# Dont4rootMe/beast_tokenizer

Measured on AMD Instinct MI355X. Metric: trajectories/sec encode+reconstruct (B=4096,T=50,DoF=14), higher is better.
Workload: dtype f32 (fp32 MFMA fit, int64 tokens); 1 GPU; BEASTBsplineTokenizer encode->reconstruct_traj, num_dof=14 num_basis=10 seq_len=50 vocab=256 degree_p=4; global_batch=4096, per_gpu_batch=4096, seq_len=50, parallelism=dp1

## Files before the change

### beast_tokenizer_amd/csrc/codec.hip

```cpp
#include <hip/hip_runtime.h>

#include <atomic>

#include <algorithm>
#include <cstdlib>

#include "common.h"
#include "launch.h"
#include "codec_device.h"
#include "codec_encode.h"
#include "codec_reconstruct.h"
#include "codec_roundtrip.h"

namespace {

constexpr int MAX_T = 256;
constexpr int MAX_N = 16;
constexpr int MAX_D = 64;

bool g_generic_only = false;

int g_block_waves = 0;
bool wide_blocks(int64_t ntiles, const Queue& q) {
  if (g_block_waves == 4 || g_block_waves == 7 || g_block_waves == 8) return g_block_waves != 4;
// ... 67 lines not shown
    case 2: return enc_smem<2>(T, Tp, Dl, D, N, nkinds).total;
    case 4: return enc_smem<4>(T, Tp, Dl, D, N, nkinds).total;
    default: return enc_smem<8>(T, Tp, Dl, D, N, nkinds).total;
  }
}

int launch_encode(EncArgs a, int T, int D, int nj, int N, const Queue& q) {
  const int64_t traj_bytes = (int64_t)T * a.row_elems * 4;
  const bool contiguous = a.sd == 1 && a.st == a.row_elems && a.sb == (int64_t)T * a.row_elems &&
                          (((uintptr_t)a.traj) & 15) == 0 && ((int64_t)T * a.row_elems) % 4 == 0;
  static const int forced = [] {
    const char* e = getenv("BEAST_ENC_TBT");
    return e ? atoi(e) : 0;
  }();
  int tbt = 8;
  while (tbt > 1 && tbt * traj_bytes > 32 * 1024) tbt >>= 1;
  const bool fast = contiguous && tbt * traj_bytes <= 32 * 1024;
  if (!fast) {
    tbt = 8;
    while (tbt > 1 && enc_smem_total(tbt, T, D, D, N, nj < D ? 2 : 1) > 160 * 1024) tbt >>= 1;
  }
  if (forced == 1 || forced == 2 || forced == 4 || (forced == 8 && fast)) tbt = std::min(tbt, forced);
  BEAST_REQUIRE(!a.traj_list || (fast && a.list_rows % tbt == 0),
                "encode list: rows must be contiguous and rows per batch a multiple of %d", tbt);
  if (fast && tbt == 8 && !g_generic_only && T == 50 && N == 10 && a.row_elems == D) {
    int rc = 0;
    const bool out16 = (((uintptr_t)a.params_out | (uintptr_t)a.tokens_out) & 15) == 0;
    if (!a.traj_list && enc_v() && out16 &&
        with_fixed_shape<false>(D, nj, false, rc, [&](auto sh) { return launch_encode_v<decltype(sh)>(a, q); }))
      return rc;
    if (with_fixed_shape<true>(D, nj, wide_blocks((a.B + 7) / 8, q), rc, [&](auto sh) {
          return launch_encode_t<8, decltype(sh)>(a, T, D, nj, N, true, q);
        }))
      return rc;
  }
  switch (tbt) {
    case 1: return launch_encode_t<1, DynShape>(a, T, D, nj, N, fast, q);
    case 2: return launch_encode_t<2, DynShape>(a, T, D, nj, N, fast, q);
    case 4: return launch_encode_t<4, DynShape>(a, T, D, nj, N, fast, q);
    default: return launch_encode_t<8, DynShape>(a, T, D, nj, N, fast, q);
  }
}

template <int TBT, int KS, int RT, class S = DynShape>
int launch_rec_ks(RecArgs a, int D, int nj, const Queue& q) {
  const RecSmem L = rec_smem<TBT, KS, RT>(a.Tout, D, a.g.N, a.ndo, nj < D ? 2 : 1, a.lut_n);
  BEAST_REQUIRE_CODE(L.total <= 160 * 1024, BEAST_E_UNSUPPORTED, "reconstruct tile needs %d B of LDS", L.total);
  const int64_t grid = grid_for(a.ntiles, L.total, q.dev);
  if constexpr (KS == 0) {
    mark_launch(launch_mark(FAM_REC_ROWS, TBT, NWAVES, 0, false, false, L.stage, false));
    return launch<k_reconstruct_rows<TBT>>((unsigned)grid, NTHREADS, L.total, q, "k_reconstruct_rows", a);
  } else {
    mark_launch(launch_mark(S::fixed ? FAM_REC_SPEC : FAM_REC_MFMA, TBT, S::W, KS, false, RT > 0, true, S::W == 7));
    return launch<k_reconstruct<TBT, KS, RT, S>>(
        (unsigned)grid, S::W * 64, L.total, q, "k_reconstruct",
        a.ntokens ? static_cast<const void*>(a.ntokens) : static_cast<const void*>(a.tokens), a.B, a.ntokens ? 4 : 8, a);
  }
}

template <int TBT, int RT>
int launch_rec_mfma(RecArgs a, int D, int nj, int N, const Queue& q) {
  switch ((N + 3) / 4) {
    case 1: return launch_rec_ks<TBT, 1, RT>(a, D, nj, q);
    case 2: return launch_rec_ks<TBT, 2, RT>(a, D, nj, q);
    case 3: return launch_rec_ks<TBT, 3, RT>(a, D, nj, q);
    default: return launch_rec_ks<TBT, 4, RT>(a, D, nj, q);
  }
}

bool rec_v(const RecArgs& a, const Queue& q) {
  return (g_block_waves == 8 || (g_block_waves == 0 && a.ntiles <= 2 * (int64_t)cu_count(q.dev))) &&
         a.params_out == nullptr && a.ntokens == nullptr && (((uintptr_t)a.pos_out) & 15) == 0;
}

template <class S>
int launch_rec_v(RecArgs a, const Queue& q) {
  constexpr int KS = (S::N + 3) / 4;
  constexpr RvSmem L = rv_smem<S>(S::NJ < S::D ? 2 : 1);
  static_assert(L.total <= (RV_WR <= 8 ? 64 : 160) * 1024, "k_reconstruct_v LDS");
  a.tbt = RV_WR;
  a.ntiles = (a.B + RV_WR - 1) / RV_WR;
  const bool lat = a.B <= 16 * (int64_t)cu_count(q.dev);
  mark_launch(launch_mark(FAM_REC_V, RV_WR, RV_WR, KS, false, true, true, lat));
  const RecVArgs v{a.w_min, a.w_max, a.basis, a.dof_dst, a.init_p, a.init_p_src, a.pos_out, a.tok_offset,
                   a.init_p_sb, a.vocab, a.lut_n, a.phases};
  const unsigned grid = (unsigned)a.ntiles;
  return lat ? launch<k_reconstruct_v<KS, S, LAT_SP>>(grid, RV_WR * 64, L.total, q, "k_reconstruct_v", a.tokens, a.B, 8, v)
             : launch<k_reconstruct_v<KS, S, 0>>(grid, RV_WR * 64, L.total, q, "k_reconstruct_v", a.tokens, a.B, 8, v);
}

template <int TBT>
bool rec_mfma_fits(int Tout, int D, int N, int ndo, int lut_n) {
  return rec_smem<TBT, 4, 0>(Tout, D, N, ndo, 2, lut_n).total <= 112 * 1024;
}

template <int TBT>
int launch_reconstruct(RecArgs a, int D, int nj, int N, bool shared, const Queue& q) {
  a.g = make_geom<TBT>(D, nj, N, 1);
  a.ntiles = (a.B + TBT - 1) / TBT;
  a.tbt = TBT;
  a.fd_row = make_fd((uint32_t)(a.Tout * a.ndo));
  a.lut_n = (a.ntokens == nullptr && a.vocab <= LUT_MAX) ? a.vocab : 0;
  const bool pos = a.pos_out != nullptr;
  const bool mfma = shared && pos && rec_mfma_fits<TBT>(a.Tout, D, N, a.ndo, a.lut_n);
  if (!mfma) return launch_rec_ks<TBT, 0, 0>(a, D, nj, q);
  if (a.Tout <= 16 * RT_REG) {
    if (!g_generic_only && N == 10 && a.Tout == 50 && a.ndo == D) {
      int rc = 0;
      const bool wide = wide_blocks(a.ntiles, q);
      if (wide && rec_v(a, q) &&
          with_fixed_shape<false>(D, nj, false, rc, [&](auto sh) { return launch_rec_v<decltype(sh)>(a, q); }))
        return rc;
      if (with_fixed_shape<true>(D, nj, wide, rc, [&](auto sh) {
            return launch_rec_ks<TBT, 3, RT_REG, decltype(sh)>(a, D, nj, q);
          }))
        return rc;
    }
    return launch_rec_mfma<TBT, RT_REG>(a, D, nj, N, q);
  }
  return launch_rec_mfma<TBT, 0>(a, D, nj, N, q);
}

template <class S, int WF>
int launch_roundtrip(const float* traj, int64_t B, RtArgs a, int W, const Queue& q) {
  const RtSmem L = rt_smem(a.T, a.D, a.N, a.nj < a.D ? 2 : 1, W, a.lut_n);
  BEAST_REQUIRE_CODE(L.total <= 160 * 1024, BEAST_E_UNSUPPORTED, "round trip tile needs %d B of LDS", L.total);
  const int64_t grid = grid_for((B + W - 1) / W, L.total, q.dev);
  return launch<k_roundtrip<S, WF>>((unsigned)grid, (unsigned)(W * 64), (unsigned)L.total, q, "k_roundtrip", traj, B, a);
}

template <class S>
int launch_roundtrip_fixed(const float* traj, int64_t B, const RtArgs& a, const Queue& q) {
  return B <= RT_W * (int64_t)cu_count(q.dev) ? launch_roundtrip<S, RT_W>(traj, B, a, RT_W, q)
                                              : launch_roundtrip<S, RT_W_BULK>(traj, B, a, RT_W_BULK, q);
}

}

extern "C" int beast_encode_f32(const float* traj, int64_t B, int T, int64_t sb, int64_t st, int64_t sd,
                                int row_elems, int D, int n_joint, const int32_t* dof_src, const float* proj,
                                int N, const float* w_min, const float* w_max, int vocab, int64_t tok_offset,
                                float* params_out, int64_t* tokens_out, void* stream) {
  BEAST_REQUIRE(traj && dof_src && proj, "beast_encode_f32: null input pointer");
  BEAST_REQUIRE(params_out || tokens_out, "beast_encode_f32: no output requested");
  BEAST_REQUIRE(T >= 1 && T <= MAX_T, "seq_len T=%d outside [1, %d]", T, MAX_T);
  BEAST_REQUIRE(N >= 1 && N <= MAX_N, "num_basis N=%d outside [1, %d]", N, MAX_N);
  BEAST_REQUIRE(D >= 1 && D <= MAX_D && n_joint >= 0 && n_joint <= D, "bad DoF split D=%d n_joint=%d", D, n_joint);
  BEAST_REQUIRE(row_elems >= 1, "row_elems must be >= 1");
  BEAST_REQUIRE(!tokens_out || (w_min && w_max && vocab >= 2), "quantisation needs w_min/w_max and vocab >= 2");
  BEAST_REQUIRE(B >= 0, "batch size B=%lld must be >= 0", (long long)B);
  if (B == 0) return BEAST_OK;
  EncArgs a{};
  a.traj = traj; a.B = B; a.sb = sb; a.st = st; a.sd = sd; a.row_elems = row_elems; a.vocab = vocab;
  a.phases = debug_phases(); a.dof_src = dof_src; a.proj = proj; a.w_min = w_min; a.w_max = w_max;
  a.tok_offset = tok_offset; a.params_out = params_out; a.tokens_out = reinterpret_cast<long long*>(tokens_out);
  Queue q;
  if (const int rc = queue_of(stream, q, "beast_encode_f32")) return rc;
  return launch_encode(a, T, D, n_joint, N, q);
}

extern "C" int beast_encode_list_f32(const float* const* traj_list, int nbatch, int64_t rows_per_batch, int T,
                                     int row_elems, int D, int n_joint, const int32_t* dof_src, const float* proj,
                                     int N, float* params_out, void* stream) {
  BEAST_REQUIRE(traj_list && dof_src && proj && params_out, "beast_encode_list_f32: null pointer");
  BEAST_REQUIRE(nbatch >= 0 && rows_per_batch >= 0, "beast_encode_list_f32: negative sizes");
  BEAST_REQUIRE(rows_per_batch % 8 == 0, "rows_per_batch=%lld is not a multiple of 8", (long long)rows_per_batch);
  BEAST_REQUIRE(T >= 1 && T <= MAX_T, "seq_len T=%d outside [1, %d]", T, MAX_T);
  BEAST_REQUIRE(N >= 1 && N <= MAX_N, "num_basis N=%d outside [1, %d]", N, MAX_N);
// ... 139 lines not shown
```

### beast_tokenizer_amd/csrc/codec_device.h

```cpp
#pragma once

#include <hip/hip_runtime.h>

#include <algorithm>
#include <cstdint>
#include <type_traits>

#include "common.h"

namespace {

constexpr int NTHREADS = 256;
constexpr int NWAVES = NTHREADS / 64;

typedef float float4_t __attribute__((ext_vector_type(4)));

__host__ __device__ constexpr int round_up(int x, int m) { return (x + m - 1) / m * m; }

struct FastDiv {
  uint32_t d, m;
};
inline FastDiv make_fd(uint32_t d) {
  FastDiv f;
  f.d = d;
// ... 21 lines not shown
__device__ __forceinline__ void st16(void* p, float4 v) {
  st16<SP>(p, u32x4_t{__float_as_uint(v.x), __float_as_uint(v.y), __float_as_uint(v.z), __float_as_uint(v.w)});
}
template <int SP>
__device__ __forceinline__ void st16(void* p, long long a, long long b) {
  st16<SP>(p, u32x4_t{(unsigned)a, (unsigned)((unsigned long long)a >> 32), (unsigned)b,
                      (unsigned)((unsigned long long)b >> 32)});
}

template <int NT = NTHREADS, int SP = 0>
__device__ __forceinline__ void store_out(float* __restrict__ dst, const float* __restrict__ src, int count) {
  if ((((uintptr_t)src | (uintptr_t)dst) & 15) == 0) {
    const int n4 = count >> 2;
    const float4* s4 = reinterpret_cast<const float4*>(src);
    float4* d4 = reinterpret_cast<float4*>(dst);
    for (int i = threadIdx.x; i < n4; i += NT) st16<SP>(d4 + i, s4[i]);
    for (int i = (n4 << 2) + threadIdx.x; i < count; i += NT) dst[i] = src[i];
  } else {
    for (int i = threadIdx.x; i < count; i += NT) dst[i] = src[i];
  }
}

typedef __attribute__((address_space(3))) void lds_void;

template <int NT = NTHREADS>
__device__ __forceinline__ void dma16(void* lds, const void* g, int n16) {
  const int tid = threadIdx.x, wb = tid & ~63;
  for (int base = 0; base < n16; base += NT) {
    if (base + wb < n16)
      __builtin_amdgcn_global_load_lds(static_cast<const uint4*>(g) + min(base + tid, n16 - 1),
                                       (lds_void*)(static_cast<uint4*>(lds) + base + wb), 16, 0, 0);
  }
}

template <int NT = NTHREADS>
__device__ __forceinline__ void dma4(void* lds, const void* g, int n) {
  const int tid = threadIdx.x, wb = tid & ~63;
  for (int base = 0; base < n; base += NT) {
    if (base + wb < n)
      __builtin_amdgcn_global_load_lds(static_cast<const uint32_t*>(g) + min(base + tid, n - 1),
                                       (lds_void*)(static_cast<uint32_t*>(lds) + base + wb), 4, 0, 0);
  }
}

template <class V>
__device__ __forceinline__ void pin(V& v) {
  asm volatile("" : "+v"(v));
}

template <int NT = NTHREADS>
__device__ __forceinline__ void stage_rows(void* lds, const void* base, int64_t B, int esz, int64_t b0, int per,
                                           int tbt) {
  const int nb = (int)min<int64_t>(B - b0, tbt);
  const char* src = static_cast<const char*>(base) + b0 * per * esz;
  const int bytes = nb * per * esz;
  if ((bytes & 15) == 0 && (((uintptr_t)src) & 15) == 0) dma16<NT>(lds, src, bytes >> 4);
  else dma4<NT>(lds, src, bytes >> 2);
}


using beast::wave_sync;

__device__ __forceinline__ void lut_fill(float* lut, int lut_n, float vm1, int nt) {
  for (int t = threadIdx.x; t < lut_n; t += nt) lut[t] = __fdiv_rn((float)t, vm1);
}

__device__ __forceinline__ float tok_f32(long long t) { return (float)t; }

template <int NQ, class Tok>
__device__ __forceinline__ void lut_quotients(const Tok (&t)[NQ], const float* lut, int lut_n, float vm1,
                                              float (&nrm)[NQ]) {
  using U = std::make_unsigned_t<Tok>;
  bool far = false;
#pragma unroll
  for (int u = 0; u < NQ; ++u) {
    const bool in = (U)t[u] < (U)lut_n;
    far = far | !in;
    nrm[u] = lut[in ? (int)t[u] : 0];
  }
  if (far) {
#pragma unroll
    for (int u = 0; u < NQ; ++u)
      if (!((U)t[u] < (U)lut_n)) nrm[u] = __fdiv_rn(tok_f32(t[u]), vm1);
  }
}

template <bool Q3>
__device__ __forceinline__ int slot_row(int lk, int u) {
  return (!Q3 || u < 2 || lk < 2) ? (4 * lk | u) : 4 * (lk - 2) + 3;
}
template <bool Q3, int NQ>
__device__ __forceinline__ void slot_values(const float (&p4)[4], float (&p)[NQ]) {
  if constexpr (Q3) {
    const auto sw = __builtin_amdgcn_permlane32_swap(__float_as_uint(p4[2]), __float_as_uint(p4[3]), false, false);
    p[0] = p4[0]; p[1] = p4[1]; p[2] = __uint_as_float(sw[0]);
  } else {
#pragma unroll
    for (int r = 0; r < 4; ++r) p[r] = p4[r];
  }
}

template <int SP, int N16, class T>
__device__ __forceinline__ void wave_copy_out(T* g, const T* img, int lane) {
  constexpr int K = 16 / sizeof(T);
#pragma unroll
  for (int u = 0; u < (N16 + 63) / 64; ++u) {
    const int i = u * 64 + lane;
    if (i < N16) st16<SP>(g + K * i, *reinterpret_cast<const u32x4_t*>(img + K * i));
  }
}

#ifdef BEAST_STAMPS
__device__ unsigned long long g_stamps[2][16][16];
#define STAMP(k, i)                                                                              \
  do {                                                                                           \
    if (blockIdx.x == 0 && (threadIdx.x & 63) == 0) g_stamps[k][threadIdx.x >> 6][i] = __builtin_amdgcn_s_memtime(); \
  } while (0)
__device__ unsigned long long g_bstamps[2][4096][4];
#define BSTAMP(k, i)                                                                             \
  do {                                                                                           \
    if (threadIdx.x == 0 && blockIdx.x < 4096) {                                                 \
      g_bstamps[k][blockIdx.x][i] = __builtin_amdgcn_s_memrealtime();                            \
      if (i == 0)                                                                                \
        g_bstamps[k][blockIdx.x][2] = ((unsigned long long)__builtin_amdgcn_s_getreg(0xF814) << 32) | \
                                      (unsigned)__builtin_amdgcn_s_getreg(0xF804);               \
    }                                                                                            \
  } while (0)
#else
#define STAMP(k, i) do { } while (0)
#define BSTAMP(k, i) do { } while (0)
#endif

struct Geom {
  int D, nj, N, T, Tp, per;
  int nq0, nq;
  FastDiv fd_nj, fd_ng, fd_per, fd_N, fd_D, fd_nq;
};

template <int TBT>
inline Geom make_geom(int D, int nj, int N, int T) {
  Geom g;
  g.D = D; g.nj = nj; g.N = N; g.T = T; g.Tp = round_up(T, 4); g.per = N * D;
  const int ng = D - nj;
  g.nq0 = (TBT * nj + 15) / 16;
  g.nq = g.nq0 + (TBT * ng + 15) / 16;
  g.fd_nj = make_fd(std::max(nj, 1));
  g.fd_ng = make_fd(std::max(ng, 1));
  g.fd_per = make_fd(g.per);
  g.fd_N = make_fd(N);
  g.fd_D = make_fd(D);
  g.fd_nq = make_fd(std::max(g.nq, 1));
  return g;
}

template <int SD, int SNJ, int SN, int ST, int SDL, int SW = NWAVES>
struct Shape {
  static constexpr int D = SD, NJ = SNJ, N = SN, T = ST, DL = SDL;
  static constexpr int W = SW;
  static constexpr bool fixed = SD > 0;
};
using DynShape = Shape<0, 0, 0, 0, 0>;

template <class S>
struct Dims {
  int D, nj, ng, N, T, Tp, per;
  __device__ __forceinline__ Dims(const Geom& g)
// ... 38 lines not shown
```

### beast_tokenizer_amd/csrc/codec_reconstruct.h

```cpp
#pragma once

#include "codec_device.h"
#include "codec_encode.h"

namespace {

struct RecArgs {
  const long long* tokens;
  const float* ntokens;
  int64_t B, ntiles, tok_offset, basis_sb, init_p_sb;
  int vocab, Tout, ndo, phases, lut_n, tbt;
  const float* w_min;
  const float* w_max;
  const float* basis;
  const int32_t* dof_dst;
  const float* init_p;
  const int32_t* init_p_src;
  float* params_out;
  float* pos_out;
  Geom g;
  FastDiv fd_row;
};

struct RecVArgs {
  const float* w_min;
  const float* w_max;
  const float* basis;
  const int32_t* dof_dst;
  const float* init_p;
  const int32_t* init_p_src;
  float* pos_out;
  int64_t tok_offset, init_p_sb;
  int vocab, lut_n, phases;
};

constexpr int LUT_MAX = 4096;
constexpr int RT_REG = 4;

__device__ __forceinline__ float rec_weight(const RecArgs& a, const unsigned char* tokl, int e, int k,
                                            const float* wlo, const float* whi, const float* lut, float vm1) {
  const float lo = wlo[k], hi = whi[k];
  if (a.ntokens) return beast::denormalize_one(reinterpret_cast<const float*>(tokl)[e], lo, hi);
  const long long t[1] = {reinterpret_cast<const long long*>(tokl)[e] - a.tok_offset};
  float nrm[1];
  lut_quotients(t, lut, a.lut_n, vm1, nrm);
  return beast::dequantize_quotient(nrm[0], lo, hi);
}

template <int KS>
__device__ __forceinline__ void rec_weights(const RecArgs& a, const unsigned char* tokl, int j, int d, int lk,
                                            int N, int D, int per, const float* wlo, const float* whi,
                                            const float* lut, float vm1, float (&w)[KS]) {
  float lo[KS], hi[KS];
  int e[KS];
#pragma unroll
  for (int ks = 0; ks < KS; ++ks) {
    const int n = min(lk * KS + ks, N - 1), k = d * N + n;
    e[ks] = j * per + n * D + d;
    lo[ks] = wlo[k];
    hi[ks] = whi[k];
  }
  if (a.ntokens) {
#pragma unroll
    for (int ks = 0; ks < KS; ++ks)
      w[ks] = beast::denormalize_one(reinterpret_cast<const float*>(tokl)[e[ks]], lo[ks], hi[ks]);
    return;
  }
  long long t[KS];
#pragma unroll
  for (int ks = 0; ks < KS; ++ks) t[ks] = reinterpret_cast<const long long*>(tokl)[e[ks]] - a.tok_offset;
  float nrm[KS];
  lut_quotients(t, lut, a.lut_n, vm1, nrm);
#pragma unroll
  for (int ks = 0; ks < KS; ++ks) w[ks] = beast::dequantize_quotient(nrm[ks], lo[ks], hi[ks]);
}

struct RecSmem {
  int phi, tok, wlo, whi, lut, dst, out, pb, pmap, col2d, total;
  int Np4, RTR;
  bool stage;
};

template <int TBT, int KS, int RT>
__host__ __device__ inline RecSmem rec_smem(int Tout, int D, int N, int ndo, int nkinds, int lut_n) {
  RecSmem s;
  const int per = N * D;
  s.Np4 = KS ? 4 * KS : round_up(N, 4);
  s.RTR = KS ? round_up(Tout, 64) : Tout;
  int o = 0;
  s.phi = o;   o += KS ? (RT == 0 ? round_up(nkinds * s.RTR * s.Np4 * 4, 16) : round_up(nkinds * Tout * N * 4, 1024)) : 0;
  s.tok = o;   o += round_up(TBT * per * 8, 1024);
  s.wlo = o;   o += round_up(per * 4, 256);
  s.whi = o;   o += round_up(per * 4, 256);
  s.lut = o;   o += round_up(lut_n * 4, 16);
  s.dst = o;   o += round_up(D * 4, 256);
  s.pb = o;    o += KS ? 0 : round_up(TBT * D * s.Np4 * 4, 16);
  s.pmap = o;  o += KS ? 0 : round_up(per * 2, 16);
  s.col2d = o; o += KS ? 0 : round_up(ndo * 4, 16);
  const int outb = round_up(TBT * s.RTR * ndo * 4, 16);
  s.stage = KS ? true : (o + outb) <= 96 * 1024;
  s.out = o;   o += s.stage ? outb : 0;
  s.total = o;
  return s;
}

template <int NT = NTHREADS>
__device__ __forceinline__ void rec_params_out(const RecArgs& a, const unsigned char* tokl, int64_t b0, int nb,
                                               const float* wlo, const float* whi, const float* lut, float vm1) {
  const Geom& g = a.g;
  const int per = g.per, D = g.D, N = g.N;
  float* pout = a.params_out + b0 * per;
  for (int e = threadIdx.x; e < nb * per; e += NT) {
    const uint32_t j = fdiv(e, g.fd_per);
    const int k = e - j * per;
    const uint32_t d = fdiv(k, g.fd_N);
    const int n = k - d * N;
// ... 93 lines not shown
    if constexpr (RT > 0) {
      if (tile == blockIdx.x) {
#pragma unroll
        for (int kd = 0; kd < 2; ++kd)
#pragma unroll
          for (int rt = 0; rt < RT; ++rt)
#pragma unroll
            for (int ks = 0; ks < KS; ++ks) {
              const int t = rt * 16 + lr, n = lk * KS + ks;
              const float x = phi[(min(kd, nkinds - 1) * Tout + min(t, Tout - 1)) * N + min(n, N - 1)];
              phr[kd][rt][ks] = (t < Tout && n < N && kd < nkinds) ? x : 0.0f;
            }
      }
    }
    if (a.params_out != nullptr) rec_params_out<NT>(a, tokl, b0, nb, wlo, whi, lut, vm1);

    for (int q = wave; (a.phases & 2) && q < nq; q += NW) {
      int j, d, kind;
      bool ok;
      tile_col<TBT>(g, m, q, lr, j, d, kind, ok);
      ok = ok && j < nb;
      float w[KS];
      rec_weights<KS>(a, tokl, j, d, lk, N, D, per, wlo, whi, lut, vm1, w);
#pragma unroll
      for (int ks = 0; ks < KS; ++ks) w[ks] = (ok && lk * KS + ks < N) ? w[ks] : 0.0f;
      if (a.init_p != nullptr && lk == 0 && ok && d < nj)
        w[0] = a.init_p[(b0 + j) * a.init_p_sb + a.init_p_src[d]];
      float* oc = ob + (j * RTR + lk * 4) * ndo + min(max(dst[d], 0), ndo - 1);
      if constexpr (RT > 0) {
        float4_t acc[RT];
#pragma unroll
        for (int i = 0; i < RT; ++i) acc[i] = float4_t{0.0f, 0.0f, 0.0f, 0.0f};
#pragma unroll
        for (int ks = 0; ks < KS; ++ks)
#pragma unroll
          for (int i = 0; i < RT; ++i)
            acc[i] = __builtin_amdgcn_mfma_f32_16x16x4f32(kind ? phr[1][i][ks] : phr[0][i][ks], w[ks], acc[i], 0,
                                                          0, 0);
        if (ok) {
#pragma unroll
          for (int i = 0; i < RT; ++i)
#pragma unroll
            for (int r = 0; r < 4; ++r) oc[(i * 16 + r) * ndo] = acc[i][r];
        }
      } else {
        const float* Ph = phi + (kind * RTR + lr) * Np4 + lk * KS;
        for (int rt = 0; rt < RTR / 16; rt += 4) {
          float av[4][KS];
#pragma unroll
          for (int i = 0; i < 4; ++i)
#pragma unroll
            for (int ks = 0; ks < KS; ++ks) av[i][ks] = Ph[((rt + i) * 16) * Np4 + ks];
          float4_t acc[4];
#pragma unroll
          for (int i = 0; i < 4; ++i) acc[i] = float4_t{0.0f, 0.0f, 0.0f, 0.0f};
#pragma unroll
          for (int ks = 0; ks < KS; ++ks)
#pragma unroll
            for (int i = 0; i < 4; ++i)
              acc[i] = __builtin_amdgcn_mfma_f32_16x16x4f32(av[i][ks], w[ks], acc[i], 0, 0, 0);
          if (ok) {
#pragma unroll
            for (int i = 0; i < 4; ++i)
#pragma unroll
              for (int r = 0; r < 4; ++r) oc[((rt + i) * 16 + r) * ndo] = acc[i][r];
          }
        }
      }
    }
    if (tile == blockIdx.x) STAMP(1, 5);
    __syncthreads();
    if (tile == blockIdx.x) STAMP(1, 6);
    if (a.phases & 4) rec_store<S>(a, a.pos_out + b0 * (int64_t)Tout * ndo, ob, nb, RTR);
    if (tile == blockIdx.x) STAMP(1, 7);
  }
#ifdef BEAST_STAMPS
  __builtin_amdgcn_s_waitcnt(0);
  STAMP(1, 8);
  BSTAMP(1, 1);
#endif
}


struct RvSmem {
  int tok, wlo, whi, phi, zero, lut, wimg, img, total;
};
template <class S>
__host__ __device__ constexpr int rv_zero_bytes(int nkinds) {
  return round_up(((nkinds - 1) * S::T + round_up(S::T, 16)) * S::N * 4, 16);
}
template <class S>
__host__ __device__ constexpr RvSmem rv_smem(int nkinds) {
  RvSmem s{};
  constexpr int per = S::D * S::N;
  int o = 0;
  s.tok = o;  o += round_up(RV_WR * per * 8, 1024);
  s.wlo = o;  o += round_up(per * 4, 256);
  s.whi = o;  o += round_up(per * 4, 256);
  s.phi = o;  o += round_up(nkinds * S::T * S::N * 4, 1024);
  s.zero = o; o += rv_zero_bytes<S>(nkinds);
  s.lut = o;  o += round_up(LUT_MAX * 4, 16);
  s.wimg = o; o += round_up(RV_WR * (per + 4) * 4, 16);
  s.img = o;  o += RV_WR * round_up(S::T * S::D * 4, 16);
  s.total = o;
  return s;
}

typedef __attribute__((address_space(4))) const int32_t const_i32;

template <int KS, class S, int SP>
__global__ __launch_bounds__(RV_WR * 64) void k_reconstruct_v(const void* __restrict__ tsrc, int64_t B, int esz,
                                                             RecVArgs a) {
  static_assert(S::fixed && S::T > 0 && S::T <= 64 && S::D <= 16 && S::DL == S::D && 4 * KS >= S::N,
                "per-trajectory reconstruct: fixed shape, T <= 64, D <= 16, ndo == D");
  constexpr int NT = RV_WR * 64, D = S::D, N = S::N, T = S::T, per = D * N;
  constexpr int NJ = S::NJ;
  constexpr int nkinds = NJ < D ? 2 : 1;
  constexpr RvSmem L = rv_smem<S>(nkinds);
  constexpr int RV_IMG = round_up(T * D * 4, 16) / 4;
  constexpr int WIMG = per + 4;
  constexpr int NU = (per + 63) / 64;
  constexpr int NTT = (T + 15) / 16;
  static_assert((T * D) % 4 == 0, "per-trajectory reconstruct: whole 16-byte rows");
  extern __shared__ __attribute__((aligned(16))) unsigned char smem[];
  float* wlo = reinterpret_cast<float*>(smem + L.wlo);
  float* whi = reinterpret_cast<float*>(smem + L.whi);
  float* phi = reinterpret_cast<float*>(smem + L.phi);
  float* lut = reinterpret_cast<float*>(smem + L.lut);
  const int tid = threadIdx.x, wave = __builtin_amdgcn_readfirstlane(tid >> 6), lane = tid & 63;
  const int64_t b0 = (int64_t)blockIdx.x * RV_WR;
  STAMP(1, 0);
  BSTAMP(1, 0);
  stage_rows<NT>(smem + L.tok, tsrc, B, esz, b0, per, RV_WR);
  STAMP(1, 9);
  dma4<NT>(wlo, a.w_min, per);
  dma4<NT>(whi, a.w_max, per);
  {
    constexpr int pbytes = nkinds * T * N * 4;
    if ((pbytes & 15) == 0 && (((uintptr_t)a.basis) & 15) == 0) dma16<NT>(phi, a.basis, pbytes >> 4);
    else dma4<NT>(phi, a.basis, pbytes >> 2);
  }
  const float vm1 = (float)(a.vocab - 1);
  lut_fill(lut, a.lut_n, vm1, NT);
  for (int i = tid; i < rv_zero_bytes<S>(nkinds) / 4; i += NT) reinterpret_cast<float*>(smem + L.zero)[i] = 0.0f;
  STAMP(1, 12);
  const int j = wave;
  const int nb = (int)min<int64_t>(RV_WR, B - b0);
  int te[NU], kb[NU], wk[NU];
#pragma unroll
  for (int u = 0; u < NU; ++u) {
    const int e = u * 64 + lane, ec = min(e, per - 1);
    const int n = ec / D, d = ec - n * D, k = d * N + n;
    te[u] = L.tok + (j * per + ec) * 8;
    kb[u] = k * 4;
    wk[u] = L.wimg + (j * WIMG + (e < per ? k : per)) * 4;
    pin(te[u]); pin(kb[u]); pin(wk[u]);
  }
  const int c = lane & 15, kk = lane >> 4;
  int dsrc = -1;
  const_i32* dof_dst = (const_i32*)a.dof_dst;
#pragma unroll
  for (int d = 0; d < D; ++d) dsrc = dof_dst[d] == c ? d : dsrc;
  const bool row_ok = dsrc >= 0;
  const int dd = row_ok ? dsrc : 0;
  int wa[KS];
  unsigned am[nkinds];
#pragma unroll
  for (int s2 = 0; s2 < KS; ++s2) {
    const int n = kk * KS + s2;
    wa[s2] = (row_ok && n < N) ? L.wimg + (j * WIMG + dd * N + n) * 4 : L.zero;
    pin(wa[s2]);
  }
#pragma unroll
  for (int kd = 0; kd < nkinds; ++kd) {
    am[kd] = (nkinds == 1 || ((dd < NJ) == (kd == 0))) ? ~0u : 0u;
    pin(am[kd]);
  }
  int pa[KS], pt[KS];
#pragma unroll
  for (int s2 = 0; s2 < KS; ++s2) {
    const int n = kk * KS + s2, tl = (NTT - 1) * 16 + c;
    pa[s2] = n < N ? L.phi + (c * N + n) * 4 : L.zero;
    pt[s2] = (n < N && tl < T) ? L.phi + (c * N + n) * 4 : L.zero;
    pin(pa[s2]); pin(pt[s2]);
  }
  int ia = L.img + (j * RV_IMG + c * D + 4 * kk) * 4;
  pin(ia);
  __syncthreads();
  STAMP(1, 2);
  if (j >= nb) return;
  long long tv[NU];
  float lo[NU], hi[NU];
#pragma unroll
  for (int u = 0; u < NU; ++u) {
    tv[u] = *reinterpret_cast<const long long*>(smem + te[u]) - a.tok_offset;
    lo[u] = *reinterpret_cast<const float*>(smem + L.wlo + kb[u]);
    hi[u] = *reinterpret_cast<const float*>(smem + L.whi + kb[u]);
  }
  float nrm[NU];
  lut_quotients(tv, lut, a.lut_n, vm1, nrm);
#pragma unroll
  for (int u = 0; u < NU; ++u) {
    float w = beast::dequantize_quotient(nrm[u], lo[u], hi[u]);
    if (u == 0 && a.init_p != nullptr && lane < NJ)
      w = a.init_p[(b0 + j) * a.init_p_sb + a.init_p_src[lane]];
    *reinterpret_cast<float*>(smem + wk[u]) = w;
  }
  wave_sync();
  STAMP(1, 3);
  float4_t acc[NTT];
#pragma unroll
  for (int tt = 0; tt < NTT; ++tt) acc[tt] = float4_t{0.0f, 0.0f, 0.0f, 0.0f};
  float wv[KS];
#pragma unroll
  for (int s2 = 0; s2 < KS; ++s2) wv[s2] = *reinterpret_cast<const float*>(smem + wa[s2]);
#pragma unroll
  for (int kd = 0; kd < nkinds; ++kd) {
    float bv[NTT][KS];
#pragma unroll
    for (int tt = 0; tt < NTT; ++tt)
#pragma unroll
      for (int s2 = 0; s2 < KS; ++s2)
        bv[tt][s2] = *reinterpret_cast<const float*>(smem + (tt * 16 + 15 < T ? pa[s2] : pt[s2]) +
                                                     (kd * T + tt * 16) * N * 4);
#pragma unroll
    for (int s2 = 0; s2 < KS; ++s2) {
      const float ak = nkinds == 1 ? wv[s2] : __uint_as_float(__float_as_uint(wv[s2]) & am[kd]);
#pragma unroll
      for (int tt = 0; tt < NTT; ++tt)
        acc[tt] = __builtin_amdgcn_mfma_f32_16x16x4f32(ak, bv[tt][s2], acc[tt], 0, 0, 0);
    }
  }
  STAMP(1, 5);
  float* img = reinterpret_cast<float*>(smem + L.img) + j * RV_IMG;
#pragma unroll
  for (int tt = 0; tt < NTT; ++tt) {
    const int t = tt * 16 + c;
    if (t < T) {
      float* q = reinterpret_cast<float*>(smem + ia + tt * 16 * D * 4);
      if (4 * kk + 1 < D) *reinterpret_cast<float2*>(q) = make_float2(acc[tt][0], acc[tt][1]);
      else if (4 * kk < D) q[0] = acc[tt][0];
      if (4 * kk + 3 < D) *reinterpret_cast<float2*>(q + 2) = make_float2(acc[tt][2], acc[tt][3]);
      else if (4 * kk + 2 < D) q[2] = acc[tt][2];
    }
  }
  wave_sync();
  STAMP(1, 6);
  if (a.phases & 4)
    wave_copy_out<SP, T * D / 4>(reinterpret_cast<float4*>(a.pos_out + (b0 + j) * (int64_t)T * D),
                                 reinterpret_cast<const float4*>(img), lane);
  STAMP(1, 7);
#ifdef BEAST_STAMPS
  __builtin_amdgcn_s_waitcnt(0);
  STAMP(1, 8);
  BSTAMP(1, 1);
#endif
}

template <int TBT>
__global__ __launch_bounds__(NTHREADS) void k_reconstruct_rows(RecArgs a) {
  extern __shared__ __attribute__((aligned(16))) unsigned char smem[];
  const Geom& g = a.g;
  const int D = g.D, N = g.N, nj = g.nj, per = g.per;
  const int Tout = a.Tout, ndo = a.ndo;
  const bool pos = a.pos_out != nullptr;
  const RecSmem L = rec_smem<TBT, 0, 0>(Tout, D, N, ndo, (nj < D) ? 2 : 1, a.lut_n);
  const int Np4 = L.Np4;
  const unsigned char* tokl = smem + L.tok;
  float* pb = reinterpret_cast<float*>(smem + L.pb);
  float* wlo = reinterpret_cast<float*>(smem + L.wlo);
  float* whi = reinterpret_cast<float*>(smem + L.whi);
  float* lut = reinterpret_cast<float*>(smem + L.lut);
  uint16_t* pmap = reinterpret_cast<uint16_t*>(smem + L.pmap);
  int* dst = reinterpret_cast<int*>(smem + L.dst);
  int* col2d = reinterpret_cast<int*>(smem + L.col2d);
  float* ob = reinterpret_cast<float*>(smem + L.out);
  const int tid = threadIdx.x;
  const float vm1 = (float)(a.vocab - 1);

  const void* tsrc = a.ntokens ? static_cast<const void*>(a.ntokens) : static_cast<const void*>(a.tokens);
  const int esz = a.ntokens ? 4 : 8;
  if (blockIdx.x < a.ntiles) stage_rows(smem + L.tok, tsrc, a.B, esz, (int64_t)blockIdx.x * TBT, per, TBT);
  dma4(wlo, a.w_min, per);
  dma4(whi, a.w_max, per);
  if (pos) dma4(dst, a.dof_dst, D);
  lut_fill(lut, a.lut_n, vm1, NTHREADS);
  for (int r = tid; r < per; r += NTHREADS) {
    const int n = r / D, d = r - n * D;
    pmap[r] = (uint16_t)(d * Np4 + n);
// ... 53 lines not shown
```

### beast_tokenizer_amd/csrc/common.h

```cpp
#pragma once

#include <hip/hip_runtime.h>

#include <cstdarg>
#include <cstdint>
#include <cstdio>

#include "beast_hip.h"

namespace beast {

void set_error(const char* fmt, ...);
extern int64_t g_merge_lds_min;
extern int g_bpe_encode_mode;
extern int g_bpe_dedup_key_bits;
extern int g_bpe_train_host;
int hip_fail(hipError_t e, const char* what);
int comm_agree(beast_comm* comm, int rc, hipStream_t s);
int comm_max_i32(beast_comm* comm, int v, int* out, hipStream_t s);

inline hipStream_t as_stream(void* s) { return reinterpret_cast<hipStream_t>(s); }

__device__ __forceinline__ void wave_sync() {
  __builtin_amdgcn_fence(__ATOMIC_RELEASE, "wavefront");
  __builtin_amdgcn_wave_barrier();
  __builtin_amdgcn_fence(__ATOMIC_ACQUIRE, "wavefront");
}

__device__ __forceinline__ float clamp_t(float x, float lo, float hi) {
  if (lo != lo || hi != hi) return __builtin_nanf("");
  float r = (x < lo) ? lo : x;
  return (hi < r) ? hi : r;
}

__device__ __forceinline__ long long quantize_one(float p, float lo, float hi, float vm1) {
  float x = clamp_t(p, lo, hi);
  float s = __fsub_rn(hi, lo);
  s = (s < 1e-8f) ? 1e-8f : s;
  float u = __fdiv_rn(__fsub_rn(x, lo), s);
  u = (u < 0.0f) ? 0.0f : u;
  u = (1.0f < u) ? 1.0f : u;
  float r = rintf(__fmul_rn(u, vm1));
  if (r != r) return (long long)0x8000000000000000ULL;
  return (long long)r;
}

__device__ __forceinline__ int quantize_bin(float p, float lo, float hi, float vm1) {
  const float x = clamp_t(p, lo, hi);
  float s = __fsub_rn(hi, lo);
  s = (s < 1e-8f) ? 1e-8f : s;
  float u = __fdiv_rn(__fsub_rn(x, lo), s);
  u = (u < 0.0f) ? 0.0f : u;
  u = (1.0f < u) ? 1.0f : u;
  const float r = rintf(__fmul_rn(u, vm1));
  return (r != r) ? (int)0x80000000 : (int)r;
}

__device__ __forceinline__ int quantize_bin_k(float p, float lo, float hi, float k, float vm1, bool& exact) {
  const float x = __builtin_amdgcn_fmed3f(p, lo, hi);
  const float va = __fmul_rn(__fsub_rn(x, lo), k);
  const float f = __builtin_amdgcn_fractf(va);
  exact = exact | !(fabsf(__fsub_rn(f, 0.5f)) > 9.5367431640625e-7f * vm1) | (p != p);
  return (int)rintf(fminf(fmaxf(va, 0.0f), vm1));
}

__device__ __forceinline__ float quantize_scale(float lo, float hi, float vm1) {
  float s = __fsub_rn(hi, lo);
  s = (s < 1e-8f) ? 1e-8f : s;
  return __fmul_rn(vm1, __builtin_amdgcn_rcpf(s));
}

template <int NQ>
__device__ __forceinline__ void quantize_bins(const float (&p)[NQ], const float (&lo)[NQ], const float (&hi)[NQ],
                                              float vm1, int (&bin)[NQ], const float* k = nullptr) {
  bool ex = false;
#pragma unroll
  for (int u = 0; u < NQ; ++u)
    bin[u] = quantize_bin_k(p[u], lo[u], hi[u], k ? k[u] : quantize_scale(lo[u], hi[u], vm1), vm1, ex);
  if (ex) {
#pragma unroll
    for (int u = 0; u < NQ; ++u) bin[u] = quantize_bin(p[u], lo[u], hi[u], vm1);
  }
}

__device__ __forceinline__ long long widen_bin(int bin, unsigned long long offset) {
  const unsigned long long v = (bin == (int)0x80000000) ? 0x8000000000000000ULL : (unsigned long long)(long long)bin;
  return (long long)(v + offset);
}

__device__ __forceinline__ float dequantize_quotient(float n, float lo, float hi) {
  return clamp_t(__fadd_rn(__fmul_rn(n, __fsub_rn(hi, lo)), lo), lo, hi);
}
__device__ __forceinline__ float dequantize_one(long long tok, float lo, float hi, float vm1) {
  return dequantize_quotient(__fdiv_rn((float)tok, vm1), lo, hi);
}

__device__ __forceinline__ float normalize_one(float p, float lo, float hi) {
  const float x = clamp_t(p, lo, hi);
  float s = __fsub_rn(hi, lo);
  s = (s < 1e-8f) ? 1e-8f : s;
  const float u = __fdiv_rn(__fsub_rn(x, lo), s);
  return __fadd_rn(__fmul_rn(u, 2.0f), -1.0f);
}

__device__ __forceinline__ float denormalize_one(float x, float lo, float hi) {
  float c = (x < -1.0f) ? -1.0f : x;
  c = (1.0f < c) ? 1.0f : c;
  const float u = __fdiv_rn(__fsub_rn(c, -1.0f), 2.0f);
  return __fadd_rn(__fmul_rn(u, __fsub_rn(hi, lo)), lo);
}

}

#define BEAST_REQUIRE(cond, ...)                 \
  do {                                           \
    if (!(cond)) {                               \
      beast::set_error(__VA_ARGS__);             \
      return BEAST_E_INVALID;                    \
    }                                            \
  } while (0)

#define BEAST_REQUIRE_CODE(cond, code, ...)      \
  do {                                           \
    if (!(cond)) {                               \
      beast::set_error(__VA_ARGS__);             \
      return code;                               \
    }                                            \
  } while (0)

#define BEAST_HIP(call, what)                                     \
  do {                                                            \
    hipError_t _e = (call);                                       \
    if (_e != hipSuccess) return beast::hip_fail(_e, what);       \
  } while (0)

#define BEAST_TRY(...)                                            \
  do {                                                            \
    if (const int _rc = (__VA_ARGS__)) return _rc;                \
  } while (0)
```

Baseline: 463.1 million trajectories/s.

## Replace reconstruct LUT with FMA-corrected reciprocal quotient and shared lane table

In the per-trajectory reconstruct kernel, the 4096-entry LDS lookup table for token/(vocab-1) is dropped. The quotient is now computed with a host-supplied reciprocal and one FMA correction step, so the per-block LUT fill and its LDS footprint go away. The per-lane A-operand offsets and masks, formerly computed by every wave from dof_dst, are now built once by a single builder wave into a small LDS table that the other waves read after the barrier. Token-to-weight lane mapping is also reorganised around a power-of-two DoF stride. The smaller LDS total (padded to 84KB when RV_WR==16) may change occupancy, and the FMA-corrected quotient is assumed to match correctly-rounded division for vocab up to 4096.

```diff
diff --git a/beast_tokenizer_amd/csrc/codec.hip b/beast_tokenizer_amd/csrc/codec.hip
--- a/beast_tokenizer_amd/csrc/codec.hip
+++ b/beast_tokenizer_amd/csrc/codec.hip
@@ -173,8 +173,9 @@
   a.ntiles = (a.B + RV_WR - 1) / RV_WR;
   const bool lat = a.B <= 16 * (int64_t)cu_count(q.dev);
   mark_launch(launch_mark(FAM_REC_V, RV_WR, RV_WR, KS, false, true, true, lat));
+  const float vm1 = (float)(a.vocab - 1);
   const RecVArgs v{a.w_min, a.w_max, a.basis, a.dof_dst, a.init_p, a.init_p_src, a.pos_out, a.tok_offset,
-                   a.init_p_sb, a.vocab, a.lut_n, a.phases};
+                   a.init_p_sb, a.vocab, 1.0f / vm1, a.phases};
   const unsigned grid = (unsigned)a.ntiles;
   return lat ? launch<k_reconstruct_v<KS, S, LAT_SP>>(grid, RV_WR * 64, L.total, q, "k_reconstruct_v", a.tokens, a.B, 8, v)
              : launch<k_reconstruct_v<KS, S, 0>>(grid, RV_WR * 64, L.total, q, "k_reconstruct_v", a.tokens, a.B, 8, v);
diff --git a/beast_tokenizer_amd/csrc/codec_device.h b/beast_tokenizer_amd/csrc/codec_device.h
--- a/beast_tokenizer_amd/csrc/codec_device.h
+++ b/beast_tokenizer_amd/csrc/codec_device.h
@@ -127,6 +127,22 @@
 #pragma unroll
     for (int u = 0; u < NQ; ++u)
       if (!((U)t[u] < (U)lut_n)) nrm[u] = __fdiv_rn(tok_f32(t[u]), vm1);
+  }
+}
+
+template <int NQ, class Tok>
+__device__ __forceinline__ void fma_quotients(const Tok (&t)[NQ], int qn, float vm1, float r, float (&nrm)[NQ]) {
+  using U = std::make_unsigned_t<Tok>;
+  bool far = false;
+#pragma unroll
+  for (int u = 0; u < NQ; ++u) {
+    far = far | !((U)t[u] < (U)qn);
+    nrm[u] = beast::exact_quotient((float)(int)t[u], vm1, r);
+  }
+  if (far) {
+#pragma unroll
+    for (int u = 0; u < NQ; ++u)
+      if (!((U)t[u] < (U)qn)) nrm[u] = __fdiv_rn(tok_f32(t[u]), vm1);
   }
 }
 
diff --git a/beast_tokenizer_amd/csrc/codec_reconstruct.h b/beast_tokenizer_amd/csrc/codec_reconstruct.h
--- a/beast_tokenizer_amd/csrc/codec_reconstruct.h
+++ b/beast_tokenizer_amd/csrc/codec_reconstruct.h
@@ -31,7 +31,9 @@
   const int32_t* init_p_src;
   float* pos_out;
   int64_t tok_offset, init_p_sb;
-  int vocab, lut_n, phases;
+  int vocab;
+  float rinv;
+  int phases;
 };
 
 constexpr int LUT_MAX = 4096;
@@ -291,8 +293,12 @@
 }
 
 
+#ifndef BEAST_RV_BUILDER
+#define BEAST_RV_BUILDER 3
+#endif
+constexpr int RV_BUILDER = BEAST_RV_BUILDER < RV_WR ? BEAST_RV_BUILDER : RV_WR - 1;
 struct RvSmem {
-  int tok, wlo, whi, phi, zero, lut, wimg, img, total;
+  int tok, wlo, whi, phi, zero, tab, wimg, img, total;
 };
 template <class S>
 __host__ __device__ constexpr int rv_zero_bytes(int nkinds) {
@@ -308,10 +314,10 @@
   s.whi = o;  o += round_up(per * 4, 256);
   s.phi = o;  o += round_up(nkinds * S::T * S::N * 4, 1024);
   s.zero = o; o += rv_zero_bytes<S>(nkinds);
-  s.lut = o;  o += round_up(LUT_MAX * 4, 16);
+  s.tab = o;  o += 64 * 16;
   s.wimg = o; o += round_up(RV_WR * (per + 4) * 4, 16);
   s.img = o;  o += RV_WR * round_up(S::T * S::D * 4, 16);
-  s.total = o;
+  s.total = (RV_WR == 16 && o <= 84 * 1024) ? 84 * 1024 : o;
   return s;
 }
 
@@ -328,14 +334,16 @@
   constexpr RvSmem L = rv_smem<S>(nkinds);
   constexpr int RV_IMG = round_up(T * D * 4, 16) / 4;
   constexpr int WIMG = per + 4;
-  constexpr int NU = (per + 63) / 64;
+  constexpr int DP = D <= 4 ? 4 : D <= 8 ? 8 : 16;
+  constexpr int RPS = 64 / DP;
+  constexpr int NU = (N + RPS - 1) / RPS;
   constexpr int NTT = (T + 15) / 16;
   static_assert((T * D) % 4 == 0, "per-trajectory reconstruct: whole 16-byte rows");
+  static_assert(KS <= 3, "per-trajectory reconstruct: a lane-table entry holds three A-operand offsets and a mask");
   extern __shared__ __attribute__((aligned(16))) unsigned char smem[];
   float* wlo = reinterpret_cast<float*>(smem + L.wlo);
   float* whi = reinterpret_cast<float*>(smem + L.whi);
   float* phi = reinterpret_cast<float*>(smem + L.phi);
-  float* lut = reinterpret_cast<float*>(smem + L.lut);
   const int tid = threadIdx.x, wave = __builtin_amdgcn_readfirstlane(tid >> 6), lane = tid & 63;
   const int64_t b0 = (int64_t)blockIdx.x * RV_WR;
   STAMP(1, 0);
@@ -349,41 +357,27 @@
     if ((pbytes & 15) == 0 && (((uintptr_t)a.basis) & 15) == 0) dma16<NT>(phi, a.basis, pbytes >> 4);
     else dma4<NT>(phi, a.basis, pbytes >> 2);
   }
+  STAMP(1, 13);
   const float vm1 = (float)(a.vocab - 1);
-  lut_fill(lut, a.lut_n, vm1, NT);
+  const int qn = a.vocab <= beast::EXACT_QUOTIENT_MAX ? beast::EXACT_QUOTIENT_MAX : 0;
   for (int i = tid; i < rv_zero_bytes<S>(nkinds) / 4; i += NT) reinterpret_cast<float*>(smem + L.zero)[i] = 0.0f;
   STAMP(1, 12);
   const int j = wave;
   const int nb = (int)min<int64_t>(RV_WR, B - b0);
+  const int c = lane & 15, kk = lane >> 4;
+  *reinterpret_cast<float*>(smem + L.wimg + (j * WIMG + per + 1) * 4) = 0.0f;
   int te[NU], kb[NU], wk[NU];
-#pragma unroll
-  for (int u = 0; u < NU; ++u) {
-    const int e = u * 64 + lane, ec = min(e, per - 1);
-    const int n = ec / D, d = ec - n * D, k = d * N + n;
-    te[u] = L.tok + (j * per + ec) * 8;
-    kb[u] = k * 4;
-    wk[u] = L.wimg + (j * WIMG + (e < per ? k : per)) * 4;
-    pin(te[u]); pin(kb[u]); pin(wk[u]);
-  }
-  const int c = lane & 15, kk = lane >> 4;
-  int dsrc = -1;
-  const_i32* dof_dst = (const_i32*)a.dof_dst;
-#pragma unroll
-  for (int d = 0; d < D; ++d) dsrc = dof_dst[d] == c ? d : dsrc;
-  const bool row_ok = dsrc >= 0;
-  const int dd = row_ok ? dsrc : 0;
-  int wa[KS];
-  unsigned am[nkinds];
-#pragma unroll
-  for (int s2 = 0; s2 < KS; ++s2) {
-    const int n = kk * KS + s2;
-    wa[s2] = (row_ok && n < N) ? L.wimg + (j * WIMG + dd * N + n) * 4 : L.zero;
-    pin(wa[s2]);
-  }
-#pragma unroll
-  for (int kd = 0; kd < nkinds; ++kd) {
-    am[kd] = (nkinds == 1 || ((dd < NJ) == (kd == 0))) ? ~0u : 0u;
-    pin(am[kd]);
+  {
+    const int sd = lane & (DP - 1), sn = lane / DP;
+#pragma unroll
+    for (int u = 0; u < NU; ++u) {
+      const int n = sn + RPS * u;
+      const bool ok = sd < D && n < N;
+      te[u] = L.tok + (j * per + (ok ? n * D + sd : 0)) * 8;
+      kb[u] = ok ? (sd * N + n) * 4 : 0;
+      wk[u] = L.wimg + (j * WIMG + (ok ? sd * N + n : per)) * 4;
+      pin(te[u]); pin(kb[u]); pin(wk[u]);
+    }
   }
   int pa[KS], pt[KS];
 #pragma unroll
@@ -395,6 +389,25 @@
   }
   int ia = L.img + (j * RV_IMG + c * D + 4 * kk) * 4;
   pin(ia);
+  STAMP(1, 14);
+  if (wave == RV_BUILDER) {
+    int dsrc = -1;
+    const_i32* dof_dst = (const_i32*)a.dof_dst;
+#pragma unroll
+    for (int d = 0; d < D; ++d) dsrc = dof_dst[d] == c ? d : dsrc;
+    const bool row_ok = dsrc >= 0;
+    const int dd = row_ok ? dsrc : 0;
+    int ent[4] = {0, 0, 0, 0};
+#pragma unroll
+    for (int s2 = 0; s2 < KS; ++s2) {
+      const int n = kk * KS + s2;
+      ent[s2] = L.wimg + ((row_ok && n < N) ? dd * N + n : per + 1) * 4;
+    }
+    ent[3] = (nkinds == 1 || dd < NJ) ? -1 : 0;
+    *reinterpret_cast<int4*>(smem + L.tab + lane * 16) = make_int4(ent[0], ent[1], ent[2], ent[3]);
+  }
+  STAMP(1, 15);
+  STAMP(1, 1);
   __syncthreads();
   STAMP(1, 2);
   if (j >= nb) return;
@@ -406,14 +419,24 @@
     lo[u] = *reinterpret_cast<const float*>(smem + L.wlo + kb[u]);
     hi[u] = *reinterpret_cast<const float*>(smem + L.whi + kb[u]);
   }
+  const int4 ent = *reinterpret_cast<const int4*>(smem + L.tab + lane * 16);
   float nrm[NU];
-  lut_quotients(tv, lut, a.lut_n, vm1, nrm);
+  fma_quotients(tv, qn, vm1, a.rinv, nrm);
 #pragma unroll
   for (int u = 0; u < NU; ++u) {
     float w = beast::dequantize_quotient(nrm[u], lo[u], hi[u]);
     if (u == 0 && a.init_p != nullptr && lane < NJ)
       w = a.init_p[(b0 + j) * a.init_p_sb + a.init_p_src[lane]];
     *reinterpret_cast<float*>(smem + wk[u]) = w;
+  }
+  int wa[KS];
+  unsigned am[nkinds];
+  {
+    const int et[3] = {ent.x, ent.y, ent.z};
+#pragma unroll
+    for (int s2 = 0; s2 < KS; ++s2) wa[s2] = et[s2] + j * WIMG * 4;
+#pragma unroll
+    for (int kd = 0; kd < nkinds; ++kd) am[kd] = kd == 0 ? (unsigned)ent.w : ~(unsigned)ent.w;
   }
   wave_sync();
   STAMP(1, 3);
diff --git a/beast_tokenizer_amd/csrc/common.h b/beast_tokenizer_amd/csrc/common.h
--- a/beast_tokenizer_amd/csrc/common.h
+++ b/beast_tokenizer_amd/csrc/common.h
@@ -91,6 +91,13 @@
 __device__ __forceinline__ float dequantize_quotient(float n, float lo, float hi) {
   return clamp_t(__fadd_rn(__fmul_rn(n, __fsub_rn(hi, lo)), lo), lo, hi);
 }
+constexpr int EXACT_QUOTIENT_MAX = 4096;
+__device__ __forceinline__ float exact_quotient(float t, float vm1, float r) {
+  const float q0 = __fmul_rn(t, r);
+  const float e = __fmaf_rn(-q0, vm1, t);
+  return __fmaf_rn(e, r, q0);
+}
+
 __device__ __forceinline__ float dequantize_one(long long tok, float lo, float hi, float vm1) {
   return dequantize_quotient(__fdiv_rn((float)tok, vm1), lo, hi);
 }
```

Result: faster. 473.7 million trajectories/s (median of 6 runs) (+2.3%).
